# HaploConduct/HaploConduct

Measured on AMD Instinct MI355X. Metric: candidate overlaps scored/sec (edge-calc scoring pass: compute_overlap + overlap_score + admission class, candidates resident in HBM; the whole stage from the overlaps text: stage_end_to_end), higher is better.
Workload: dtype f64; 1 GPU; c3: 500000 synthetic 2x150 bp read pairs, 6 quality values (SURVEY 8(d)), 100000000 p-p candidates per GPU; read_pairs=500000, genome_len=90000, quality_alphabet=6, candidates_per_gpu=100000000, record_bytes=16, parallelism=candidate shards x1, replicated read store

## Files before the change

### haploconduct_amd/csrc/hc_api.cpp

```cpp
#include <hip/hip_runtime.h>

#include <chrono>
#include <cmath>
#include <cstdio>
#include <cstdlib>
#include <cstring>
#include <thread>
#include <array>
#include <limits>
#include <new>
#include <string>
#include <vector>

#include "../../include/hcedge.h"
#include "hc_ctx.h"
#include "host/EnvKnobs.h"
#include "host/LogP.h"

namespace env = hc::env;
using env::Knob;

static thread_local std::string g_last_error;

static int fail(int status, const std::string& what) {
// ... 412 lines not shown
        c->fetch_group = (mean_len > 600 || symbytes == 2) ? 2 : 4;
        const uint32_t lmin = c->len_p5, lmax = c->len_p95;
        uint32_t n_pairs = 0;
        for (uint32_t r = 0; r < n_reads; r++) n_pairs += read_first_seq[r + 1] - read_first_seq[r] == 2;
        const bool short_mixed_singles = n_seq && n_pairs == 0 && lmax > 2u * lmin && mean_len <= 300 && !c->view.balance;
        c->coop_fetch = !short_mixed_singles;
        if (short_mixed_singles) c->fetch_group = 2;
    }
    c->view.long_rows = (n_seq && total / n_seq > 600) ? 1u : 0u;
    return HC_OK;
}
}
}

int hc_set_reads(hc_ctx* c, const uint8_t* bases, const uint8_t* quals, const uint64_t* seq_off,
                 const uint32_t* read_first_seq, uint32_t n_reads) {
    if (!c || !seq_off || !read_first_seq) return fail(HC_ERR_ARG, "hc_set_reads: null argument");
    HC_HIP(hipSetDevice(c->device));
    const uint32_t n_seq = read_first_seq[n_reads];
    if (read_first_seq[0] != 0) return fail(HC_ERR_BAD_READ, "hc_set_reads: read_first_seq[0] != 0");
    for (uint32_t r = 0; r < n_reads; r++) {
        const uint32_t k = read_first_seq[r + 1] - read_first_seq[r];
        if (k != 1 && k != 2) return fail(HC_ERR_BAD_READ, "hc_set_reads: a read must own 1 or 2 sequences");
    }
    const uint64_t total = seq_off[n_seq];
    if (total > 0 && (!bases || !quals)) return fail(HC_ERR_ARG, "hc_set_reads: null bases/quals");
    if (seq_off[0] != 0) return fail(HC_ERR_BAD_READ, "hc_set_reads: seq_off[0] != 0");
    std::vector<uint32_t> seq_len(n_seq ? n_seq : 1);
    for (uint32_t q = 0; q < n_seq; q++) {
        if (seq_off[q + 1] <= seq_off[q])
            return fail(HC_ERR_BAD_READ, "hc_set_reads: empty sequence");
        const uint64_t len = seq_off[q + 1] - seq_off[q];
        if (len >= (1ull << 28)) return fail(HC_ERR_BAD_READ, "hc_set_reads: sequence longer than 2^28-1");
        seq_len[q] = (uint32_t)len;
    }
    uint64_t hist[256] = {0}, base_hist[256] = {0};
    {
        const unsigned T = total < (1u << 22) ? 1u : std::min(16u, std::max(1u, std::thread::hardware_concurrency()));
        std::vector<std::array<uint64_t, 512>> part(T);
        auto work = [&](unsigned t) {
            std::array<uint64_t, 512>& h = part[t];
            h.fill(0);
            const uint64_t a = total * t / T, b = total * (t + 1) / T;
            for (uint64_t i = a; i < b; i++) {
                h[quals[i]]++;
                h[256 + bases[i]]++;
            }
        };
        std::vector<std::thread> th;
        for (unsigned t = 1; t < T; t++) th.emplace_back(work, t);
        work(0);
        for (auto& x : th) x.join();
        for (unsigned t = 0; t < T; t++)
            for (int b = 0; b < 256; b++) {
                hist[b] += part[t][(size_t)b];
                base_hist[b] += part[t][256 + (size_t)b];
            }
    }
    hc::StorePlan P;
    P.seq_len = std::move(seq_len);
    P.total = total;
    int rc = hc::plan_store(c, hist, base_hist, read_first_seq, n_reads, P);
    if (rc) return rc;
    hc::release_store(c);
    hc_ctx::SrNext& N = c->srn;
    N.raw_valid = false;
    hc_scratch t_bases, t_quals, t_raw_off, t_first;
    hc_scratch &s_bases = N.keep ? N.bases : t_bases, &s_quals = N.keep ? N.quals : t_quals, &s_off = N.keep ? N.off : t_raw_off,
               &s_first = N.keep ? N.first : t_first;
    if ((rc = s_bases.ensure_exact(total ? total : 1)) || (rc = s_quals.ensure_exact(total ? total : 1)) ||
        (rc = s_off.ensure_exact(sizeof(uint64_t) * ((size_t)n_seq + 1))) || (rc = s_first.ensure_exact(sizeof(uint32_t) * ((size_t)n_reads + 1))))
        return rc;
    if (total) {
        HC_HIP(hipMemcpyAsync(s_bases.p, bases, total, hipMemcpyHostToDevice, c->stream));
        HC_HIP(hipMemcpyAsync(s_quals.p, quals, total, hipMemcpyHostToDevice, c->stream));
    }
    HC_HIP(hipMemcpyAsync(s_off.p, seq_off, sizeof(uint64_t) * ((size_t)n_seq + 1), hipMemcpyHostToDevice, c->stream));
    HC_HIP(hipMemcpyAsync(s_first.p, read_first_seq, sizeof(uint32_t) * ((size_t)n_reads + 1), hipMemcpyHostToDevice, c->stream));
    rc = hc::finish_store(c, P, s_bases.as<uint8_t>(), s_quals.as<uint8_t>(), s_off.as<uint64_t>(), s_first.as<uint32_t>(), read_first_seq, n_reads);
    if (rc) return rc;
    if (N.keep) {
        N.h_off.assign(seq_off, seq_off + n_seq + 1);
        N.h_first.assign(read_first_seq, read_first_seq + n_reads + 1);
        N.total = total;
        N.raw_valid = true;
    }
    return HC_OK;
}

static bool host_batch_is_ordered(const void* in, size_t rec_bytes, uint64_t n) {
    if (n < 2) return true;
    const uint64_t samples = n - 1 < 4096 ? n - 1 : 4096;
    const uint64_t step = (n - 2) / samples > 0 ? (n - 2) / samples : 1;
    uint64_t share = 0;
    for (uint64_t k = 0; k < samples; k++) {
        const uint32_t* a = (const uint32_t*)((const char*)in + k * step * rec_bytes);
        const uint32_t* b = (const uint32_t*)((const char*)in + (k * step + 1) * rec_bytes);
        share += (a[0] == b[0]) | (a[0] == b[1]) | (a[1] == b[0]) | (a[1] == b[1]);
    }
    return share * 2 >= samples;
}

static int ensure_sort_workspace(hc_ctx* c, uint64_t n) {
    if (4 * n * sizeof(uint32_t) <= c->d_sort.cap) return HC_OK;
    c->d_sort.release();
    c->d_sort_tmp.release();
    const size_t tmp = hc::reorder_temp_bytes((uint32_t)n);
    int rc = c->d_sort.ensure_exact(4 * n * sizeof(uint32_t));
    if (rc == HC_OK) rc = c->d_sort_tmp.ensure_exact(tmp ? tmp : 16);
    if (rc) c->d_sort.release();
    return rc;
}

}

static constexpr uint64_t kLocalityMinCandidates = 8000000;
static bool locality_wanted(uint64_t n) {
    if (env::i(Knob::LOCALITY, 1) == 0) return false;
    return n >= env::u64(Knob::LOCALITY_MIN, kLocalityMinCandidates);
}

int hc_ctx_score(hc_ctx* c, uint32_t fmt, const void* d_in, uint64_t n, void* d_out, hipStream_t s, bool reorder,
                 hc_gather_row* rows, unsigned long long* row_count, uint64_t cap, uint64_t base_index, const unsigned long long* n_dev,
                 const hc_line_rec* lines_in, hc_line_rec* lines_out, hc_bucket_ws* bucket) {
    const uint32_t cus = c->comm_reserve && c->comm_reserve < c->n_cu ? c->n_cu - c->comm_reserve : c->n_cu;
    const hc::RowSinkKind sink = !rows ? hc::RowSinkKind::none
                                       : (!lines_in && cap < 0xFFFFFFFFull ? hc::RowSinkKind::segmented : hc::RowSinkKind::unsegmented);
    const hc::ScorePlan plan = hc::plan_score_launch(c->view, c->coop_fetch, c->fetch_group, cus, n, sink);
    const bool coop = plan.kernel && plan.kernel->coop;
    const bool want_perm = reorder && n > 1 && n < (1ull << 31);
    const bool want_loc = !want_perm && !plan.bucketed && !rows && !lines_in && !bucket && fmt == HC_REC_COMPACT && coop && c->view.regular &&
                          c->loc_reads == c->view.n_reads && c->loc_reads > 1 && n > 1 && n < (1ull << 32) && locality_wanted(n);
    const bool ctx_scratch = want_perm || (plan.bucketed && !bucket) || plan.segmented || want_loc;
    if (ctx_scratch) {
        if (!c->scratch_done) HC_HIP(hipEventCreateWithFlags(&c->scratch_done, hipEventDisableTiming));
        if (c->scratch_used && c->scratch_stream != s) HC_HIP(hipStreamWaitEvent(s, c->scratch_done, 0));
    }
    const uint32_t* perm = nullptr;
    if (want_perm) {
        int rc = ensure_sort_workspace(c, n);
        if (rc) return rc;
        const size_t sort_cap = c->d_sort.cap / (4 * sizeof(uint32_t));
        uint32_t* keys_in = c->d_sort.as<uint32_t>();
        uint32_t* keys_out = keys_in + sort_cap;
        uint32_t* idx_in = keys_in + 2 * sort_cap;
        uint32_t* perm_out = keys_in + 3 * sort_cap;
        HC_HIP(hc::launch_reorder(c->view.n_reads, fmt, d_in, (uint32_t)n, keys_in, keys_out, idx_in, perm_out, c->d_sort_tmp.p,
                                  c->d_sort_tmp.cap, s));
        perm = perm_out;
    }
    const uint32_t* order_off = nullptr;
    if (want_loc) {
        const uint32_t R = c->loc_reads;
        const size_t head = ((size_t)R + 2 + (size_t)R + 1 + 1 + 3) & ~(size_t)3;
        const size_t tmp = hc::locality_index_temp_bytes(R);
        if ((head + n) * sizeof(uint32_t) > c->loc_ws.cap && c->scratch_used) HC_HIP(hipEventSynchronize(c->scratch_done));
        int rc = c->loc_ws.ensure((head + n) * sizeof(uint32_t));
        if (rc == HC_OK) rc = c->loc_tmp.ensure(tmp ? tmp : 16);
        if (rc) return rc;
        uint32_t* flag = c->loc_ws.as<uint32_t>();
        uint32_t* bounds = flag + 1;
        uint32_t* starts = bounds + R + 2;
        uint32_t* lperm = c->loc_ws.as<uint32_t>() + head;
        HC_HIP(hc::launch_locality_index(c->loc_order.as<uint32_t>(), R, d_in, n, n_dev, bounds, starts, flag, lperm, c->loc_tmp.p, tmp, s));
        perm = lperm;
        order_off = flag;
    }
    hc::ScoreParams prm = c->params;
    prm.rec_fmt = fmt;
    prm.pad = 0;
    prm.n_dev = n_dev;
    prm.order_off = order_off;
    hc::ScoreBuffers buf{rows, row_count, cap, base_index, lines_in, lines_out};
    buf.started = (rows && !lines_in) ? c->d_started.as<unsigned long long>() : nullptr;
    if (plan.bucketed) {
        hc_bucket_ws* ws = bucket ? bucket : &c->bucket;
        int rc = ws->ensure(n);
        if (rc) return rc;
        buf.bucket_perm = ws->perm();
        buf.bucket_queue = ws->queue();
    }
    if (plan.segmented) {
        buf.seg_total_rows = 2 * cap + hc::kSinkMaxGroups * 512;
        if (buf.seg_total_rows * sizeof(hc_gather_row) > c->sink_rows.cap && c->scratch_used) HC_HIP(hipEventSynchronize(c->scratch_done));
        int rc = c->sink_rows.ensure(buf.seg_total_rows * sizeof(hc_gather_row));
        if (rc) return rc;
        if (!c->sink_counts.p) {
            if ((rc = c->sink_counts.ensure((hc::kSinkMaxGroups + 2) * sizeof(uint32_t))) != HC_OK) return rc;
            HC_HIP(hipMemsetAsync(c->sink_counts.p, 0, (hc::kSinkMaxGroups + 2) * sizeof(uint32_t), s));
        }
        if (c->sink_dirty) {
            HC_HIP(hipMemsetAsync(c->sink_counts.as<uint32_t>() + hc::kSinkMaxGroups, 0, 2 * sizeof(uint32_t), s));
            c->sink_dirty = false;
        }
        buf.seg_buf = c->sink_rows.as<hc_gather_row>();
        buf.seg_count = c->sink_counts.as<uint32_t>();
        buf.spill_turn = &c->sink_turn;
    }
    uint32_t started_groups = 0;
    const hipError_t le = hc::launch_score(plan, c->view, prm, c->d_lut.as<double>(), d_in, n, (hc_result_rec*)d_out, perm, buf, s, &started_groups);
    if (le != hipSuccess) {
        if (plan.segmented) c->sink_dirty = true;
        return hc::set_last_error(HC_ERR_HIP, std::string("launch_score: ") + hipGetErrorString(le));
    }
    if (buf.started) c->started_target += started_groups;
    if (ctx_scratch) {
        HC_HIP(hipEventRecord(c->scratch_done, s));
        c->scratch_stream = s;
        c->scratch_used = true;
    }
    return HC_OK;
}

extern "C" {

int hc_set_reorder(hc_ctx* c, int mode) {
    if (!c || mode < HC_REORDER_NEVER || mode > HC_REORDER_AUTO) return fail(HC_ERR_ARG, "hc_set_reorder: bad argument");
    c->reorder_mode = mode;
    return HC_OK;
}

int hc_get_locality_order(hc_ctx* c, uint32_t* out, uint64_t cap, uint64_t* n) {
    if (!c || !n || (cap && !out)) return fail(HC_ERR_ARG, "hc_get_locality_order: bad argument");
    *n = c->have_reads ? c->loc_reads : 0;
    const uint64_t k = std::min<uint64_t>(cap, *n);
    if (k) {
        HC_HIP(hipSetDevice(c->device));
        HC_HIP(hipMemcpy(out, c->loc_order.p, k * sizeof(uint32_t), hipMemcpyDeviceToHost));
    }
    return HC_OK;
}

int hc_score_batch_device(hc_ctx* c, const void* d_in, uint64_t n, void* d_out, void* hip_stream) {
    if (!c) return fail(HC_ERR_ARG, "hc_score_batch_device: null context");
    if (!c->have_reads) return fail(HC_ERR_STATE, "hc_score_batch_device: hc_set_reads has not been called");
    if (n == 0) return HC_OK;
    if (!d_in || !d_out) return fail(HC_ERR_ARG, "hc_score_batch_device: null buffer");
    HC_HIP(hipSetDevice(c->device));
    hipStream_t s = hip_stream ? (hipStream_t)hip_stream : c->stream;
    return hc_ctx_score(c, HC_REC_FULL, d_in, n, d_out, s, c->reorder_mode == HC_REORDER_ALWAYS, nullptr, nullptr, 0, 0);
}

int hc_score_cands_device(hc_ctx* c, const void* d_in, uint64_t n, void* d_out, void* hip_stream) {
    if (!c) return fail(HC_ERR_ARG, "hc_score_cands_device: null context");
    if (!c->have_reads) return fail(HC_ERR_STATE, "hc_score_cands_device: hc_set_reads has not been called");
    if (n == 0) return HC_OK;
    if (!d_in || !d_out) return fail(HC_ERR_ARG, "hc_score_cands_device: null buffer");
    HC_HIP(hipSetDevice(c->device));
    hipStream_t s = hip_stream ? (hipStream_t)hip_stream : c->stream;
    return hc_ctx_score(c, HC_REC_COMPACT, d_in, n, d_out, s, c->reorder_mode == HC_REORDER_ALWAYS, nullptr, nullptr, 0, 0);
}

void hc_pack_cands(const hc_overlap_rec* in, uint64_t n, hc_cand_rec* out) {
    for (uint64_t i = 0; i < n; i++) {
        const hc_overlap_rec& r = in[i];
        const uint32_t p1 = r.pos1 < HC_CAND_POS_MASK ? r.pos1 : HC_CAND_POS_MASK;
        const uint32_t p2 = r.pos2 < HC_CAND_POS_MASK ? r.pos2 : HC_CAND_POS_MASK;
        const uint32_t oc = r.ord == '-' ? 0u : (r.ord == '1' ? 1u : (r.ord == '2' ? 2u : 3u));
        out[i].read1 = r.read1;
        out[i].read2 = r.read2;
        out[i].pos1_bits = p1 | (r.ori1 ? 1u << 28 : 0u) | (r.ori2 ? 1u << 29 : 0u) | (oc << 30);
        out[i].pos2_bits = p2;
    }
}

int hc_synchronize(hc_ctx* c) {
    if (!c) return fail(HC_ERR_ARG, "hc_synchronize: null context");
    HC_HIP(hipSetDevice(c->device));
    HC_HIP(hipStreamSynchronize(c->stream));
    return HC_OK;
}

static int ensure_workspace(hc_ctx* c, uint64_t n) {
    const int rc = c->d_in.ensure_exact(n * sizeof(hc_overlap_rec));
    return rc ? rc : c->d_out.ensure_exact(n * sizeof(hc_result_rec));
}

static int score_host(hc_ctx* c, const char* who, uint32_t fmt, const void* in, uint64_t n, hc_result_rec* out) {
    if (!c) return fail(HC_ERR_ARG, std::string(who) + ": null context");
    if (!c->have_reads) return fail(HC_ERR_STATE, std::string(who) + ": hc_set_reads has not been called");
    if (n == 0) return HC_OK;
    if (!in || !out) return fail(HC_ERR_ARG, std::string(who) + ": null buffer");
    HC_HIP(hipSetDevice(c->device));
    int rc = ensure_workspace(c, n);
    if (rc) return rc;
    const size_t rb = fmt == HC_REC_COMPACT ? sizeof(hc_cand_rec) : sizeof(hc_overlap_rec);
    HC_HIP(hipMemcpyAsync(c->d_in.p, in, n * rb, hipMemcpyHostToDevice, c->stream));
    bool reorder = c->reorder_mode == HC_REORDER_ALWAYS;
    if (c->reorder_mode == HC_REORDER_AUTO && n >= 4096) reorder = !host_batch_is_ordered(in, rb, n);
    rc = hc_ctx_score(c, fmt, c->d_in.p, n, c->d_out.p, c->stream, reorder, nullptr, nullptr, 0, 0);
    if (rc) return rc;
    HC_HIP(hipMemcpyAsync(out, c->d_out.p, n * sizeof(hc_result_rec), hipMemcpyDeviceToHost, c->stream));
    HC_HIP(hipStreamSynchronize(c->stream));
    return HC_OK;
}

int hc_score_batch(hc_ctx* c, const hc_overlap_rec* in, uint64_t n, hc_result_rec* out) {
    return score_host(c, "hc_score_batch", HC_REC_FULL, in, n, out);
}

int hc_score_cands(hc_ctx* c, const hc_cand_rec* in, uint64_t n, hc_result_rec* out) {
    return score_host(c, "hc_score_cands", HC_REC_COMPACT, in, n, out);
}

int hc_host_alloc(hc_ctx* c, void** ptr, uint64_t bytes) {
    if (!c || !ptr) return fail(HC_ERR_ARG, "hc_host_alloc: null argument");
    *ptr = nullptr;
    HC_HIP(hipSetDevice(c->device));
    HC_HIP(hipHostMalloc(ptr, bytes ? bytes : 1, hipHostMallocDefault));
    return HC_OK;
}

int hc_host_free(hc_ctx* c, void* ptr) {
    if (!c) return fail(HC_ERR_ARG, "hc_host_free: null context");
    if (ptr) HC_HIP(hipHostFree(ptr));
    return HC_OK;
}
// ... 253 lines not shown
```

### haploconduct_amd/csrc/hc_ctx.h

```cpp
#pragma once
#include <hip/hip_runtime.h>

#include <atomic>
#include <utility>
#include <string>
#include <vector>

#include "../../include/hcedge.h"
#include "../../include/hcsr.h"
#include "hc_device.h"
#include "hc_overlap_finder.h"
#include "hc_scratch.h"

namespace hc {
hipError_t launch_encode(uint32_t symbytes, const uint8_t* bases, const uint8_t* quals, const uint64_t* raw_off,
                         const uint64_t* seq_off, const uint32_t* rc_delta, const uint8_t* qmap, uint32_t n_seq, uint32_t K, void* sym,
                         uint8_t* seq_bad, const uint32_t* read_first_seq, uint32_t n_reads, ReadDesc* descs, uint32_t slot_align,
                         hipStream_t stream);
struct ScoreKernel {
    bool coop;
    uint32_t symbytes, lg, wg;
    uint32_t group;
    bool bal;
    uint32_t depth;
    bool wq;
    const void* fn;
    const char* name;
};
enum class RowSinkKind { none, segmented, unsegmented };
struct ScorePlan {
    const ScoreKernel* kernel = nullptr;
    const ScoreKernel* staged = nullptr;
    uint32_t blocks = 0;
    size_t lds = 0;
    size_t lds_form = 0;
    uint32_t waves_per_cu = 0;
    bool bucketed = false;
    bool segmented = false;
};
ScorePlan plan_score_launch(const StoreView& st, bool coop_fetch, int lane_group, uint32_t n_cu, uint64_t n, RowSinkKind sink);
struct ScoreBuffers {
    hc_gather_row* rows = nullptr;
    unsigned long long* row_count = nullptr;
    uint64_t cap = 0, base_index = 0;
    const hc_line_rec* lines_in = nullptr;
    hc_line_rec* lines_out = nullptr;
    uint32_t* bucket_perm = nullptr;
    uint32_t* bucket_queue = nullptr;
    hc_gather_row* seg_buf = nullptr;
    uint32_t* seg_count = nullptr;
    uint64_t seg_total_rows = 0;
    uint32_t* spill_turn = nullptr;
    unsigned long long* started = nullptr;
};
hipError_t launch_score(const ScorePlan& plan, const StoreView& st, ScoreParams prm, const double* lut_g, const void* in, uint64_t n,
                        hc_result_rec* out, const uint32_t* perm, const ScoreBuffers& buf, hipStream_t stream, uint32_t* started_groups);
hipError_t set_score_kernel_lds_limit();
std::string describe_score_kernel(const StoreView& st, bool coop_fetch, int lane_group, uint32_t n_cu, uint64_t n);
size_t compact_temp_bytes(uint32_t n);
hipError_t launch_compact(const hc_result_rec* res, uint32_t n, uint32_t* idx_out, unsigned long long* count_out, void* temp,
                          size_t temp_bytes, hipStream_t stream);
hipError_t launch_narrow_payload(const void* in32, uint64_t cap, void* out24, uint32_t n_cu, hipStream_t stream);
hipError_t launch_pack_rows(const hc_result_rec* res, const uint32_t* idx, const unsigned long long* count, uint64_t cap, uint64_t base,
                            hc_gather_row* rows, uint32_t n_cu, hipStream_t stream);
hipError_t launch_pack_header(const unsigned long long* count, hc_gather_row* header, hipStream_t stream);
hipError_t launch_gather_results(const hc_result_rec* res, const uint32_t* idx, const unsigned long long* count,
                                 hc_result_rec* out, uint32_t n_cu, hipStream_t stream);
size_t reorder_temp_bytes(uint32_t n);
hipError_t launch_reorder(uint32_t n_reads, uint32_t fmt, const void* in, uint32_t n, uint32_t* keys_in, uint32_t* keys_out,
                          uint32_t* idx_in, uint32_t* perm_out, void* temp, size_t temp_bytes, hipStream_t stream);
hipError_t launch_count_positions(const StoreView& st, uint32_t min_read_len, uint32_t fmt, const void* in, uint64_t n,
                                  unsigned long long* totals, hipStream_t stream);
hipError_t launch_kept_rows(const hc_result_rec* res, uint64_t n, const unsigned long long* n_dev, uint64_t base_index, uint32_t* tile_cnt,
                            uint32_t* tile_off, hc_gather_row* rows, uint64_t cap, unsigned long long* count, const hc_line_rec* lines_in,
                            hc_line_rec* lines_out, hipStream_t stream, const uint32_t* text_tally = nullptr,
                            unsigned long long* text_counters = nullptr);
hipError_t launch_flush_text_rows(const void* rows, void* rows_mapped, const void* lines, void* lines_mapped, const unsigned long long* count,
                                  uint64_t cap, const unsigned long long* counters, unsigned long long* counters_mapped, uint32_t n_cu,
                                  hipStream_t stream);
hipError_t launch_comm_gate(const unsigned long long* started, unsigned long long target, uint32_t timeout_us, hipStream_t stream);
hipError_t launch_flush_rows(const void* src, void* dst_mapped, const unsigned long long* count, uint64_t cap, uint32_t row_bytes, uint32_t n_cu,
                             hipStream_t stream);

size_t locality_order_temp_bytes(uint32_t n_reads);
hipError_t launch_locality_order(const uint8_t* bases, const uint64_t* raw_off, const uint32_t* read_first_seq, uint32_t n_reads, uint64_t* keys_a,
                                 uint64_t* keys_b, uint32_t* idx, uint32_t* order_out, void* temp, size_t temp_bytes, hipStream_t stream);
size_t locality_index_temp_bytes(uint32_t n_reads);
hipError_t launch_locality_index(const uint32_t* order, uint32_t n_reads, const void* in, uint64_t n, const unsigned long long* n_dev, uint32_t* bounds,
                                 uint32_t* start, uint32_t* flag, uint32_t* perm, void* temp, size_t temp_bytes, hipStream_t stream);

Band threshold_band(double T, int log2_width);
struct StorePlan {
    std::vector<uint32_t> seq_len;
    uint64_t total = 0;
    uint8_t qmap[256];
    uint32_t K = 0, symbytes = 0, slot_align = 0;
    uint64_t nsym = 0;
    std::vector<uint64_t> sym_off;
    std::vector<uint32_t> rc_delta;
    std::vector<double> lut;
    bool any_bad_base = false;
};
}
struct hc_ctx;
namespace hc {
int plan_store(hc_ctx* c, const uint64_t* hist, const uint64_t* base_hist, const uint32_t* read_first_seq, uint32_t n_reads, StorePlan& P);
void release_store(hc_ctx* c);
int finish_store(hc_ctx* c, const StorePlan& P, const uint8_t* d_bases, const uint8_t* d_quals, const uint64_t* d_raw_off, const uint32_t* d_first,
                 const uint32_t* read_first_seq, uint32_t n_reads);
bool build_log_table_u16(const std::vector<int>& phred, double mismatch_setting, std::vector<double>& lut);
}

struct hc_bucket_ws {
    hc_scratch mem;
    int ensure(uint64_t n) { return mem.ensure((n + 16) * sizeof(uint32_t)); }
    uint32_t* queue() const { return mem.as<uint32_t>(); }
    uint32_t* perm() const { return mem.as<uint32_t>() + 16; }
};

struct hc_ctx {
    hc_settings settings;
    int device = 0;
    uint32_t n_cu = 256;
    bool coop_fetch = true;
    int fetch_group = 4;
    hipStream_t stream = nullptr;
    hipStream_t text_copy_stream[4] = {nullptr, nullptr, nullptr, nullptr};
    std::atomic<uint32_t> text_copy_next{0};
    hipEvent_t ev0 = nullptr, ev1 = nullptr;
    bool have_reads = false;
    hc_scratch d_sym, d_reads, d_lut, d_inv_n;
    uint32_t len_p5 = 0, len_p95 = 0;
    uint64_t store_bytes = 0;
    hc::StoreView view{};
    hc::ScoreParams params{};
    std::vector<hc::SeqRef> seq_refs;
    bool singles_first = true;
    hc_scratch finder_scratch[24], ingest_scratch[12];
    hc_scratch h_ingest[2] = {hc_scratch(hipHostMallocDefault), hc_scratch(hipHostMallocDefault)};
    hc_scratch h_sfo_text[3] = {hc_scratch(hipHostMallocDefault), hc_scratch(hipHostMallocDefault),
                                hc_scratch(hipHostMallocDefault)};
    hc_scratch d_found;
    uint64_t n_found = 0;
    hc_scratch d_found_lines;
    double found_err = -1;
    uint32_t found_min = 0, found_flags = 0;
    bool found_valid = false;
    hc_scratch d_in, d_out;
    hc_scratch d_totals;
    int reorder_mode = HC_REORDER_AUTO;
    hc_scratch d_sort, d_sort_tmp;
    hc_bucket_ws bucket;
    hc_scratch loc_order, loc_ws, loc_tmp;
    uint32_t loc_reads = 0;
    hc_scratch sink_rows, sink_counts;
    uint32_t sink_turn = 0;
    bool sink_dirty = false;
    uint32_t comm_reserve = 0;
    hc_scratch d_started;
    unsigned long long started_target = 0;

    hipEvent_t scratch_done = nullptr;
    hipStream_t scratch_stream = nullptr;
    bool scratch_used = false;
    hc_scratch d_compact_tmp, d_compact_idx, d_compact_res;
    hc_scratch id_table, id_keys;
    uint64_t id_size = 0;
    int id_shift = 0, id_direct = 1;
    bool have_ids = false;
    struct Graph {
        hc_scratch adm, E, key0, key1, idx0, idx1, keep, incl, tied, counters, surv, k32a, k32b, k64a, k64b, tmp_idx, o_out, o_in,
            out_off, in_off, edges_out, in_nodes, vtx, temp, tied_list;
        hc_scratch edges_next, seq_next, out_off_next, in_nodes_next, in_off_next, clean_temp, incl_vtx, incl_off, incl_edges;
        uint64_t n_groups = 0, n_group_edges = 0;
        bool have_groups = false;
        hc_scratch branching, tip_reads, read_geom;
        uint64_t n_branching = 0, n_tip_reads = 0;
        uint64_t n_vertices = 0, n_edges = 0, n_tied = 0;
        uint64_t n_appended = 0;
        bool valid = false;
        hc_scratch h_stage[2] = {hc_scratch(hipHostMallocDefault), hc_scratch(hipHostMallocDefault)};
        hipEvent_t stage_free[2] = {nullptr, nullptr};
        int stage_turn = 0;
    } graph;
    struct GraphText {
        hc_scratch sizes, keep, counters, temp, text;
        uint64_t n_bytes = 0;
        bool valid = false;
        void drop() { valid = false, n_bytes = 0; }
    } graph_text;
    struct SrTables {
        hc_scratch terms, qbyte, table;
        bool valid = false, has_nan = false;
        double min_qual = 0;
        uint8_t q_of[128];
    };
    uint8_t sr_qbyte[128];
    struct Sr {
        hc_scratch layouts, members, mem, info, len, off, temp, seq, qual, late, host_cols, counter;
        SrTables tables;
        hc_scratch patches;
        bool kept_valid = false;
        uint64_t kept_bytes = 0;
    } sr;
    struct SrNext {
        bool keep = false, raw_valid = false;
        hc_scratch bases, quals, off, first;
        uint64_t total = 0;
        std::vector<uint64_t> h_off;
        std::vector<uint32_t> h_first;
        hc_scratch next_bases, next_quals, next_off, next_first;
        hc_scratch entries, status, cnt, bytes, cnt_off, byte_off, temp, hist, extra_seq, extra_qual;
    } srn;
    struct SrSelf {
        hc_scratch seq, qual, pairs, skip, qmap, lut, inv_n, res, len, off, mpos, temp, out_seq, out_qual;
        hc_scratch check, segs, stage_seq, stage_qual;
        SrTables tables;
    } sr_self;
    struct SrEdge {
        hc_scratch targets, pairs, vread, vfwd, status, lay_cnt, mem_cnt, first, mem_off, layouts, members, who, sub, temp;
    } sr_edge;
    struct SrClique {
        hc_scratch off, nodes, vread, vfwd, key_in, key, hit, slot, ecnt, eoff, sel, sub, failkey, base_rank, type, geom, ext, deg, rec_off, lay0,
            pl_first, status, lay_cnt, first, mem_cnt, mem_off, pl, pl_total, pl_filter, ekey_in, ekey, eval_in, eval, ekey2, eval2, slotpos, fmem, fvert, fend,
            fused, out_layouts, out_members, out_vertex, out_used, out_filter, uflag, uoff, temp;
        bool filter_on_host = false;
    } sr_clique;
    struct SrMergeNext {
        hc_scratch pairs, pair_status, first_layout, layouts, members, lay_status, out_off, sub, v_read, v_fwd, incl, tip_reads;
        hc_scratch entries, status, cnt, bytes, key, rank, overlap_pos, n_clique, visited, rewrite;
        hc_scratch t_kind, t_id, t_v_state, t_nodes, t_srs, t_sr_pair, t_clique_cnt, t_clique_off, t_clique_nodes, t_sub_off, t_sub, t_tips, temp;
    } sr_mn;
};

namespace hc {
int sr_consensus_begin(hc_ctx* c, uint64_t* out_off, uint64_t* n_bytes, hc_sr_stats* stats);
int sr_consensus_room(hc_ctx* c, const hc_sr_settings* settings, uint64_t n_layouts, uint64_t n_members);
int sr_consensus_run(hc_ctx* c, const char* me, uint64_t n_layouts, uint64_t n_members, const hc_sr_settings* settings, int32_t* ret, uint32_t* status,
                     uint64_t* out_off, uint8_t* cons_seq, uint8_t* cons_qual, uint64_t cap, uint64_t* n_bytes, hc_sr_stats* stats, bool* ret_late);
}

int hc_ctx_score(hc_ctx* c, uint32_t fmt, const void* d_in, uint64_t n, void* d_out, hipStream_t s, bool reorder,
// ... 6 lines not shown
```

### haploconduct_amd/csrc/hc_locality.hip

```cpp
#include <hip/hip_runtime.h>
#include <stdint.h>

#include "../../include/hcedge.h"
#include "hc_prims.h"

namespace hc {

namespace {

constexpr uint32_t kLocK = 16;
constexpr uint64_t kLocHashMul = 0x9E3779B97F4A7C15ull;
constexpr int kLocKeyBits = 44;
constexpr uint64_t kLocNoKey = (1ull << kLocKeyBits) - 1;
constexpr uint32_t kLocSamples = 1u << 16;

__device__ __forceinline__ uint32_t base_code(uint8_t b) {
    return b == 'C' ? 1u : (b == 'G' ? 2u : (b == 'T' ? 3u : 0u));
}

__global__ __launch_bounds__(256) void locality_key_kernel(const uint8_t* __restrict__ bases, const uint64_t* __restrict__ raw_off,
                                                           const uint32_t* __restrict__ read_first_seq, uint32_t n_reads,
                                                           uint64_t* __restrict__ keys, uint32_t* __restrict__ idx) {
    const uint32_t r = blockIdx.x * blockDim.x + threadIdx.x;
    if (r >= n_reads) return;
    const uint32_t q = read_first_seq[r];
    const uint64_t off = raw_off[q], len = raw_off[q + 1] - off;
    uint64_t best = kLocNoKey;
    uint32_t kmer = 0;
    for (uint64_t j = 0; j < len; j++) {
        kmer = (kmer << 2) | base_code(bases[off + j]);
        if (j + 1 >= kLocK) {
            const uint64_t h = ((uint64_t)kmer * kLocHashMul) >> (64 - kLocKeyBits);
            best = h < best ? h : best;
        }
    }
    keys[r] = best;
    idx[r] = r;
}

__device__ __forceinline__ uint32_t hot_read(const void* in, uint64_t i, uint32_t n_reads) {
    const uint2 p = *((const uint2*)((const hc_cand_rec*)in + i));
    const uint32_t h = p.x < p.y ? p.x : p.y;
    return h < n_reads ? h : n_reads;
}

__global__ __launch_bounds__(256) void locality_bounds_kernel(const void* __restrict__ in, uint64_t n, const unsigned long long* __restrict__ n_dev,
                                                              uint32_t n_reads, uint32_t* __restrict__ bounds, uint32_t* __restrict__ flag) {
    const uint64_t ne = n_dev ? (*n_dev < n ? *n_dev : n) : n;
    const uint32_t t = blockIdx.x * blockDim.x + threadIdx.x;
    if (t <= n_reads + 1u) {
        uint64_t b;
        if (t == 0) b = 0;
        else if (t == n_reads + 1u) b = ne;
        else {
            uint64_t lo = 0, hi = ne;
            while (lo < hi) {
                const uint64_t mid = (lo + hi) >> 1;
                if (hot_read(in, mid, n_reads) < t) lo = mid + 1;
                else hi = mid;
            }
            b = lo;
        }
        bounds[t] = (uint32_t)b;
    }
    if (t < kLocSamples && ne >= 2) {
        const uint64_t i = (ne - 1) * t / kLocSamples;
        if (hot_read(in, i, n_reads) > hot_read(in, i + 1, n_reads)) atomicOr(flag, 1u);
    }
}

__global__ __launch_bounds__(256) void locality_lengths_kernel(const uint32_t* __restrict__ order, uint32_t n_reads, const uint32_t* __restrict__ bounds,
                                                               uint32_t* __restrict__ len, uint32_t* __restrict__ flag) {
    const uint32_t k = blockIdx.x * blockDim.x + threadIdx.x;
    if (k > n_reads) return;
    const uint32_t h = k < n_reads ? order[k] : n_reads;
    const uint32_t lo = bounds[h], hi = bounds[h + 1];
    if (hi < lo) atomicOr(flag, 1u);
    len[k] = hi >= lo ? hi - lo : 0u;
}

__global__ __launch_bounds__(256) void locality_fill_kernel(const uint32_t* __restrict__ order, uint32_t n_reads, const uint32_t* __restrict__ bounds,
                                                            const uint32_t* __restrict__ start, const uint32_t* __restrict__ flag, uint64_t n,
                                                            const unsigned long long* __restrict__ n_dev, uint32_t* __restrict__ perm) {
    const uint64_t ne = n_dev ? (*n_dev < n ? *n_dev : n) : n;
    if (*flag) {
        const uint64_t stride = (uint64_t)gridDim.x * blockDim.x;
        for (uint64_t i = (uint64_t)blockIdx.x * blockDim.x + threadIdx.x; i < ne; i += stride) perm[i] = (uint32_t)i;
        return;
    }
    const uint32_t k = (uint32_t)(((uint64_t)blockIdx.x * blockDim.x + threadIdx.x) >> 6), lane = threadIdx.x & 63u;
    if (k > n_reads) return;
    const uint32_t h = k < n_reads ? order[k] : n_reads;
    const uint32_t lo = bounds[h], len = bounds[h + 1] - lo, s = start[k];
    for (uint32_t j = lane; j < len; j += 64u)
        if ((uint64_t)s + j < ne) perm[s + j] = lo + j;
}

}

size_t locality_order_temp_bytes(uint32_t n_reads) { return prims::sort_temp_bytes(n_reads, sizeof(uint64_t), sizeof(uint32_t)); }

hipError_t launch_locality_order(const uint8_t* bases, const uint64_t* raw_off, const uint32_t* read_first_seq, uint32_t n_reads, uint64_t* keys_a,
                                 uint64_t* keys_b, uint32_t* idx, uint32_t* order_out, void* temp, size_t temp_bytes, hipStream_t stream) {
    if (n_reads == 0) return hipSuccess;
    hipLaunchKernelGGL(locality_key_kernel, dim3((n_reads + 255) / 256), dim3(256), 0, stream, bases, raw_off, read_first_seq, n_reads, keys_a, idx);
    return prims::sort_pairs(temp, temp_bytes, keys_a, keys_b, idx, order_out, n_reads, 0, kLocKeyBits, stream);
}

size_t locality_index_temp_bytes(uint32_t n_reads) { return prims::scan_temp_bytes((uint64_t)n_reads + 1, sizeof(uint32_t)); }

hipError_t launch_locality_index(const uint32_t* order, uint32_t n_reads, const void* in, uint64_t n, const unsigned long long* n_dev, uint32_t* bounds,
                                 uint32_t* start, uint32_t* flag, uint32_t* perm, void* temp, size_t temp_bytes, hipStream_t stream) {
    hipError_t e = hipMemsetAsync(flag, 0, sizeof(uint32_t), stream);
    if (e != hipSuccess) return e;
    const uint32_t threads = n_reads + 2u > kLocSamples ? n_reads + 2u : kLocSamples;
    hipLaunchKernelGGL(locality_bounds_kernel, dim3((threads + 255) / 256), dim3(256), 0, stream, in, n, n_dev, n_reads, bounds, flag);
    hipLaunchKernelGGL(locality_lengths_kernel, dim3((n_reads + 1u + 255) / 256), dim3(256), 0, stream, (const uint32_t*)order, n_reads,
                       (const uint32_t*)bounds, start, flag);
    e = prims::exclusive_sum(temp, temp_bytes, start, start, (uint64_t)n_reads + 1, stream);
    if (e != hipSuccess) return e;
    const uint64_t fill_threads = ((uint64_t)n_reads + 1) * 64;
    hipLaunchKernelGGL(locality_fill_kernel, dim3((uint32_t)((fill_threads + 255) / 256)), dim3(256), 0, stream, order, n_reads, (const uint32_t*)bounds,
                       (const uint32_t*)start, (const uint32_t*)flag, n, n_dev, perm);
    return hipGetLastError();
}

}
```

Measured before the change: 17.19 billion candidate overlaps/s.

## Replace locality index scan pipeline with tiled sums and in-block scan fill

Removes the memset, the separate lengths kernel and the library exclusive scan from the locality index build. A per-tile sums kernel now folds together the monotonicity sampling, the run-length validity check and the tile totals. The fill kernel then computes tile offsets and runs an in-block shuffle scan before writing the permutation, and it uses vectorised stores on the identity fallback. This cuts kernel launches and temp-buffer traffic, at the cost of each fill block re-summing its prefix of tile totals, which grows with tile count.

```diff
diff --git a/haploconduct_amd/csrc/hc_api.cpp b/haploconduct_amd/csrc/hc_api.cpp
--- a/haploconduct_amd/csrc/hc_api.cpp
+++ b/haploconduct_amd/csrc/hc_api.cpp
@@ -588,17 +588,15 @@
     const uint32_t* order_off = nullptr;
     if (want_loc) {
         const uint32_t R = c->loc_reads;
-        const size_t head = ((size_t)R + 2 + (size_t)R + 1 + 1 + 3) & ~(size_t)3;
-        const size_t tmp = hc::locality_index_temp_bytes(R);
+        const size_t head = (1 + (size_t)R + 2 + hc::locality_index_work_words(R) + 3) & ~(size_t)3;
         if ((head + n) * sizeof(uint32_t) > c->loc_ws.cap && c->scratch_used) HC_HIP(hipEventSynchronize(c->scratch_done));
         int rc = c->loc_ws.ensure((head + n) * sizeof(uint32_t));
-        if (rc == HC_OK) rc = c->loc_tmp.ensure(tmp ? tmp : 16);
         if (rc) return rc;
         uint32_t* flag = c->loc_ws.as<uint32_t>();
         uint32_t* bounds = flag + 1;
-        uint32_t* starts = bounds + R + 2;
+        uint32_t* work = bounds + R + 2;
         uint32_t* lperm = c->loc_ws.as<uint32_t>() + head;
-        HC_HIP(hc::launch_locality_index(c->loc_order.as<uint32_t>(), R, d_in, n, n_dev, bounds, starts, flag, lperm, c->loc_tmp.p, tmp, s));
+        HC_HIP(hc::launch_locality_index(c->loc_order.as<uint32_t>(), R, d_in, n, n_dev, bounds, work, flag, lperm, s));
         perm = lperm;
         order_off = flag;
     }
diff --git a/haploconduct_amd/csrc/hc_ctx.h b/haploconduct_amd/csrc/hc_ctx.h
--- a/haploconduct_amd/csrc/hc_ctx.h
+++ b/haploconduct_amd/csrc/hc_ctx.h
@@ -85,9 +85,9 @@
 size_t locality_order_temp_bytes(uint32_t n_reads);
 hipError_t launch_locality_order(const uint8_t* bases, const uint64_t* raw_off, const uint32_t* read_first_seq, uint32_t n_reads, uint64_t* keys_a,
                                  uint64_t* keys_b, uint32_t* idx, uint32_t* order_out, void* temp, size_t temp_bytes, hipStream_t stream);
-size_t locality_index_temp_bytes(uint32_t n_reads);
+size_t locality_index_work_words(uint32_t n_reads);
 hipError_t launch_locality_index(const uint32_t* order, uint32_t n_reads, const void* in, uint64_t n, const unsigned long long* n_dev, uint32_t* bounds,
-                                 uint32_t* start, uint32_t* flag, uint32_t* perm, void* temp, size_t temp_bytes, hipStream_t stream);
+                                 uint32_t* work, uint32_t* flag, uint32_t* perm, hipStream_t stream);
 
 Band threshold_band(double T, int log2_width);
 struct StorePlan {
diff --git a/haploconduct_amd/csrc/hc_locality.hip b/haploconduct_amd/csrc/hc_locality.hip
--- a/haploconduct_amd/csrc/hc_locality.hip
+++ b/haploconduct_amd/csrc/hc_locality.hip
@@ -13,6 +13,7 @@
 constexpr int kLocKeyBits = 44;
 constexpr uint64_t kLocNoKey = (1ull << kLocKeyBits) - 1;
 constexpr uint32_t kLocSamples = 1u << 16;
+constexpr uint32_t kLocTileRuns = 512;
 
 __device__ __forceinline__ uint32_t base_code(uint8_t b) {
     return b == 'C' ? 1u : (b == 'G' ? 2u : (b == 'T' ? 3u : 0u));
@@ -50,9 +51,12 @@
     const uint32_t t = blockIdx.x * blockDim.x + threadIdx.x;
     if (t <= n_reads + 1u) {
         uint64_t b;
-        if (t == 0) b = 0;
-        else if (t == n_reads + 1u) b = ne;
-        else {
+        if (t == 0) {
+            b = 0;
+            *flag = 0;
+        } else if (t == n_reads + 1u) {
+            b = ne;
+        } else {
             uint64_t lo = 0, hi = ne;
             while (lo < hi) {
                 const uint64_t mid = (lo + hi) >> 1;
@@ -63,37 +67,92 @@
         }
         bounds[t] = (uint32_t)b;
     }
-    if (t < kLocSamples && ne >= 2) {
-        const uint64_t i = (ne - 1) * t / kLocSamples;
-        if (hot_read(in, i, n_reads) > hot_read(in, i + 1, n_reads)) atomicOr(flag, 1u);
-    }
 }
 
-__global__ __launch_bounds__(256) void locality_lengths_kernel(const uint32_t* __restrict__ order, uint32_t n_reads, const uint32_t* __restrict__ bounds,
-                                                               uint32_t* __restrict__ len, uint32_t* __restrict__ flag) {
-    const uint32_t k = blockIdx.x * blockDim.x + threadIdx.x;
-    if (k > n_reads) return;
-    const uint32_t h = k < n_reads ? order[k] : n_reads;
-    const uint32_t lo = bounds[h], hi = bounds[h + 1];
-    if (hi < lo) atomicOr(flag, 1u);
-    len[k] = hi >= lo ? hi - lo : 0u;
+__device__ __forceinline__ uint32_t wave_sum(uint32_t v) {
+#pragma unroll
+    for (int o = 32; o > 0; o >>= 1) v += (uint32_t)__shfl_xor((int)v, o, 64);
+    return v;
+}
+
+__global__ __launch_bounds__(256) void locality_sums_kernel(const uint32_t* __restrict__ order, uint32_t n_reads, const uint32_t* __restrict__ bounds,
+                                                            const void* __restrict__ in, uint64_t n, const unsigned long long* __restrict__ n_dev,
+                                                            uint32_t* __restrict__ tile_sum, uint32_t* __restrict__ flag) {
+    __shared__ uint32_t part[4];
+    const uint64_t ne = n_dev ? (*n_dev < n ? *n_dev : n) : n;
+    uint32_t sum = 0;
+    bool bad = false;
+    if (ne >= 2)
+        for (uint32_t t = blockIdx.x * 256u + threadIdx.x; t < kLocSamples; t += gridDim.x * 256u) {
+            const uint64_t i = (ne - 1) * t / kLocSamples;
+            bad |= hot_read(in, i, n_reads) > hot_read(in, i + 1, n_reads);
+        }
+    for (uint32_t j = threadIdx.x; j < kLocTileRuns; j += 256u) {
+        const uint64_t k = (uint64_t)blockIdx.x * kLocTileRuns + j;
+        if (k > n_reads) break;
+        const uint32_t h = k < n_reads ? order[k] : n_reads;
+        const uint32_t lo = bounds[h], hi = bounds[h + 1];
+        bad |= hi < lo;
+        sum += hi >= lo ? hi - lo : 0u;
+    }
+    if (bad) atomicOr(flag, 1u);
+    sum = wave_sum(sum);
+    if ((threadIdx.x & 63u) == 0) part[threadIdx.x >> 6] = sum;
+    __syncthreads();
+    if (threadIdx.x == 0) tile_sum[blockIdx.x] = part[0] + part[1] + part[2] + part[3];
 }
 
 __global__ __launch_bounds__(256) void locality_fill_kernel(const uint32_t* __restrict__ order, uint32_t n_reads, const uint32_t* __restrict__ bounds,
-                                                            const uint32_t* __restrict__ start, const uint32_t* __restrict__ flag, uint64_t n,
-                                                            const unsigned long long* __restrict__ n_dev, uint32_t* __restrict__ perm) {
+                                                            const uint32_t* __restrict__ tile_sum, uint32_t n_tiles, const uint32_t* __restrict__ flag,
+                                                            uint64_t n, const unsigned long long* __restrict__ n_dev, uint32_t* __restrict__ perm) {
     const uint64_t ne = n_dev ? (*n_dev < n ? *n_dev : n) : n;
     if (*flag) {
-        const uint64_t stride = (uint64_t)gridDim.x * blockDim.x;
-        for (uint64_t i = (uint64_t)blockIdx.x * blockDim.x + threadIdx.x; i < ne; i += stride) perm[i] = (uint32_t)i;
+        const uint64_t stride = 4ull * gridDim.x * blockDim.x;
+        for (uint64_t i = 4ull * ((uint64_t)blockIdx.x * blockDim.x + threadIdx.x); i < ne; i += stride) {
+            if (i + 4 <= ne) *(uint4*)(perm + i) = uint4{(uint32_t)i, (uint32_t)i + 1u, (uint32_t)i + 2u, (uint32_t)i + 3u};
+            else
+                for (uint64_t p = i; p < ne; ++p) perm[p] = (uint32_t)p;
+        }
         return;
     }
-    const uint32_t k = (uint32_t)(((uint64_t)blockIdx.x * blockDim.x + threadIdx.x) >> 6), lane = threadIdx.x & 63u;
-    if (k > n_reads) return;
-    const uint32_t h = k < n_reads ? order[k] : n_reads;
-    const uint32_t lo = bounds[h], len = bounds[h + 1] - lo, s = start[k];
-    for (uint32_t j = lane; j < len; j += 64u)
-        if ((uint64_t)s + j < ne) perm[s + j] = lo + j;
+    if (blockIdx.x >= n_tiles) return;
+    __shared__ uint32_t s_start[kLocTileRuns + 1], s_lo[kLocTileRuns], part[8];
+    const uint32_t t = threadIdx.x, lane = t & 63u, wave = t >> 6;
+    uint32_t base = 0;
+    for (uint32_t j = t; j < blockIdx.x; j += 256u) base += tile_sum[j];
+    base = wave_sum(base);
+    uint32_t lo[2] = {0, 0}, len[2] = {0, 0};
+#pragma unroll
+    for (int q = 0; q < 2; ++q) {
+        const uint64_t k = (uint64_t)blockIdx.x * kLocTileRuns + 2u * t + q;
+        if (k <= n_reads) {
+            const uint32_t h = k < n_reads ? order[k] : n_reads;
+            lo[q] = bounds[h];
+            len[q] = bounds[h + 1] - lo[q];
+        }
+    }
+    uint32_t incl = len[0] + len[1];
+#pragma unroll
+    for (int o = 1; o < 64; o <<= 1) {
+        const uint32_t up = (uint32_t)__shfl_up((int)incl, o, 64);
+        if ((int)lane >= o) incl += up;
+    }
+    if (lane == 63u) part[4 + wave] = incl;
+    if (lane == 0u) part[wave] = base;
+    __syncthreads();
+    uint32_t excl = part[0] + part[1] + part[2] + part[3] + incl - (len[0] + len[1]);
+    for (uint32_t w = 0; w < wave; ++w) excl += part[4 + w];
+    s_start[2u * t] = excl;
+    s_start[2u * t + 1u] = excl + len[0];
+    s_lo[2u * t] = lo[0];
+    s_lo[2u * t + 1u] = lo[1];
+    if (t == 255u) s_start[kLocTileRuns] = excl + len[0] + len[1];
+    __syncthreads();
+    for (uint32_t r = wave; r < kLocTileRuns; r += 4u) {
+        const uint32_t s = s_start[r], len = s_start[r + 1u] - s, l0 = s_lo[r];
+        for (uint32_t j = lane; j < len; j += 64u)
+            if ((uint64_t)s + j < ne) perm[s + j] = l0 + j;
+    }
 }
 
 }
@@ -107,21 +166,18 @@
     return prims::sort_pairs(temp, temp_bytes, keys_a, keys_b, idx, order_out, n_reads, 0, kLocKeyBits, stream);
 }
 
-size_t locality_index_temp_bytes(uint32_t n_reads) { return prims::scan_temp_bytes((uint64_t)n_reads + 1, sizeof(uint32_t)); }
+static uint32_t locality_tiles(uint32_t n_reads) { return (uint32_t)(((uint64_t)n_reads + 1 + kLocTileRuns - 1) / kLocTileRuns); }
+
+size_t locality_index_work_words(uint32_t n_reads) { return locality_tiles(n_reads); }
 
 hipError_t launch_locality_index(const uint32_t* order, uint32_t n_reads, const void* in, uint64_t n, const unsigned long long* n_dev, uint32_t* bounds,
-                                 uint32_t* start, uint32_t* flag, uint32_t* perm, void* temp, size_t temp_bytes, hipStream_t stream) {
-    hipError_t e = hipMemsetAsync(flag, 0, sizeof(uint32_t), stream);
-    if (e != hipSuccess) return e;
-    const uint32_t threads = n_reads + 2u > kLocSamples ? n_reads + 2u : kLocSamples;
-    hipLaunchKernelGGL(locality_bounds_kernel, dim3((threads + 255) / 256), dim3(256), 0, stream, in, n, n_dev, n_reads, bounds, flag);
-    hipLaunchKernelGGL(locality_lengths_kernel, dim3((n_reads + 1u + 255) / 256), dim3(256), 0, stream, (const uint32_t*)order, n_reads,
-                       (const uint32_t*)bounds, start, flag);
-    e = prims::exclusive_sum(temp, temp_bytes, start, start, (uint64_t)n_reads + 1, stream);
-    if (e != hipSuccess) return e;
-    const uint64_t fill_threads = ((uint64_t)n_reads + 1) * 64;
-    hipLaunchKernelGGL(locality_fill_kernel, dim3((uint32_t)((fill_threads + 255) / 256)), dim3(256), 0, stream, order, n_reads, (const uint32_t*)bounds,
-                       (const uint32_t*)start, (const uint32_t*)flag, n, n_dev, perm);
+                                 uint32_t* work, uint32_t* flag, uint32_t* perm, hipStream_t stream) {
+    const uint32_t tiles = locality_tiles(n_reads);
+    hipLaunchKernelGGL(locality_bounds_kernel, dim3((n_reads + 2u + 255) / 256), dim3(256), 0, stream, in, n, n_dev, n_reads, bounds, flag);
+    hipLaunchKernelGGL(locality_sums_kernel, dim3(tiles), dim3(256), 0, stream, order, n_reads, (const uint32_t*)bounds, in, n, n_dev, work, flag);
+    const uint64_t wide = (n + 4095) / 4096 < 1024 ? (n + 4095) / 4096 : 1024;
+    hipLaunchKernelGGL(locality_fill_kernel, dim3(tiles > wide ? tiles : (uint32_t)wide), dim3(256), 0, stream, order, n_reads, (const uint32_t*)bounds,
+                       (const uint32_t*)work, tiles, (const uint32_t*)flag, n, n_dev, perm);
     return hipGetLastError();
 }
 
```

Result: faster. 17.44 billion candidate overlaps/s (median of 6 runs) (+1.5%).
